# zeropoolnetwork/fawkes-crypto

Hardware: AMD Instinct MI355X
Metric: Groth16 proofs/sec + MSM scalar-muls/sec, BN254, 2^25 constraints (33552553 rows = 99.99 % of the 2^25 domain) (higher is better)
Workload: dtype u32

## Files before the change

fawkes-crypto_amd/csrc/common.hpp:

```cpp
#pragma once
#include <hip/hip_runtime.h>
#include <stdint.h>
#include <stdio.h>
#include <stdlib.h>
#include <map>
#include <string>
#include <new>
#include <stdexcept>
#include <vector>
#include <functional>
#include "../../include/fawkes_hip.h"
#include "curve.hpp"

namespace fk {

struct DevBuf {
    void *p = nullptr;
    size_t cap = 0;
    hipError_t reserve(size_t bytes) {
        if (bytes <= cap) return hipSuccess;
        if (p) { hipError_t e = hipFree(p); p = nullptr; cap = 0; if (e != hipSuccess) return e; }
        size_t want = bytes + (bytes >> 3) + 256;
        hipError_t e = hipMalloc(&p, want);
        if (e != hipSuccess) { (void)hipGetLastError(); e = hipMalloc(&p, bytes); want = bytes; }
        if (e == hipSuccess) cap = want; else { p = nullptr; (void)hipGetLastError(); }
        return e;
    }
    void release() { if (p) (void)hipFree(p); p = nullptr; cap = 0; }
    template <class T> T *as() const { return (T *)p; }
};

struct NttDomain;

struct EventPair { hipEvent_t a, b; uint64_t units; };

struct MsmLane {
    hipStream_t st = nullptr;
    hipEvent_t ev_in = nullptr;
    hipEvent_t ev_sorted = nullptr;
    bool ev_sorted_valid = false;
    DevBuf digits, sorted, totals, starts, perm, overlist, tasktab, partials, s2_cnt1, s2_seg, s2_cnt2, s2_tmp_idx, s2_tmp_lo, buckets;
    DevBuf buckets2;
    const void *last_sort_scalars = nullptr; size_t last_sort_n = 0; unsigned last_sort_c = 0; bool last_merged = false;
};

struct MsmTail {
    bool active = false;
    uint32_t cb = 0, wide = 0, W = 0, nblk = 0;
    hipEvent_t done = nullptr;
    void *h_wp = nullptr;
    size_t h_cap = 0;
    DevBuf d_wp;
};
static constexpr int MSM_TAILS = 12;
static constexpr int MSM_LANES = 4;

struct QueryIdx {
    const uint8_t *d_a_aux = nullptr, *d_b_in = nullptr, *d_b_aux = nullptr;
    const uint32_t *a = nullptr, *b = nullptr;
    uint64_t n_a = 0, n_b = 0;
};

struct KeyPre {
    void *lev = nullptr;
    size_t n = 0;
    uint32_t cb = 0, wide = 0, W = 0;
};

}

struct fk_ctx {
    int device = 0;
    hipStream_t stream = nullptr;
    std::string err;
    unsigned window_bits = 0;
    unsigned ntt_threads = 512;
    std::map<uint32_t, fk::NttDomain *> domains;
    fk::MsmLane lanes[fk::MSM_LANES];
    int lane_next = 0, lane_prev = 0;
    int co_tenants = 1;
    int lanes_in_use = fk::MSM_LANES;
    fk::MsmTail tails[fk::MSM_TAILS];
    fk::DevBuf misc;
    hipStream_t aux = nullptr;
    hipEvent_t ev_aux = nullptr, ev_main = nullptr, ev_z = nullptr;
    bool defer_back = false;
    std::vector<std::function<int()>> deferred, deferred_tails;
    bool ev_z_recorded = false;
    hipEvent_t ev_acc_done = nullptr; bool ev_acc_done_valid = false;
    bool wit_active = false;
    std::function<int()> before_block;
    bool gather_on_main = false;
    struct EarlyFront { bool done = false; int tails[4] = {-1, -1, -1, -1}; const fk_key *key = nullptr; const struct fk_r1cs_dev *r1cs = nullptr; const void *d_z = nullptr; } early;
    const fk::QueryIdx *qidx = nullptr;
    int wit_tail[4] = {-1, -1, -1, -1};
    hipStream_t copy_st = nullptr;
    struct WitSlot {
        fk::DevBuf buf; hipEvent_t ready = nullptr; bool pending = false;
        hipEvent_t part = nullptr;
        bool deferred = false; const void *host_z = nullptr; size_t host_bytes = 0;
        const fk_key *key = nullptr; const struct fk_r1cs_dev *r1cs = nullptr; uint64_t r[4], s[4];
    } wslot[2];
    int wslot_next = 0;
    hipEvent_t ev_upload_gate = nullptr;
    hipEvent_t ev_chunk[16] = {nullptr};
    fk::DevBuf ntt_s1, ntt_s2, ntt_io, hbuf, sc_a, sc_b, scan_tmp, stage_a, stage_b, stage_c, stage_z, stage_d;
    std::vector<fk::EventPair> ev_acc, ev_acc2, ev_ntt;
    std::vector<hipEvent_t> ev_pool;
    uint64_t acc_adds[2] = {0, 0};
    bool stats_on = true;
    bool debug = false;
};

struct fk_key {
    uint64_t m = 0;
    uint32_t num_input = 0, num_aux = 0;
    uint64_t n_h = 0, n_l = 0, n_a = 0, n_b = 0;
    uint32_t shard_index = 0, shard_count = 1;
    uint64_t h_lo = 0, h_hi = 0, l_lo = 0, l_hi = 0, a_lo = 0, a_hi = 0, b_lo = 0, b_hi = 0;
    uint64_t b2_lo = 0, b2_hi = 0;
// ... 173 lines not shown
```

fawkes-crypto_amd/csrc/msm.hip:

```cpp
#include "common.hpp"
#include <algorithm>
#include <string.h>
#include <type_traits>

namespace fk {

static constexpr uint32_t SEG_MAX = 4096, SEG_MIN = 256;
static constexpr uint32_t SORT_THREADS = 256;

struct MsmPlan {
    size_t n;
    uint32_t c, W, B;
    uint32_t cb, wide;
    uint32_t nchunks;
    size_t chunk;
    uint32_t cap, cap_top;
    uint32_t L, T, nblk;
    uint32_t LB, nhi, nlo;
};
#ifndef FK_S2_TILE
#define FK_S2_TILE 8192
#endif
static constexpr uint32_t S2_TILE = FK_S2_TILE;
static constexpr uint32_t S2_EPT = S2_TILE / 1024;
#ifndef FK_S1_TILE
#define FK_S1_TILE 8192
#endif
static constexpr uint32_t S1_TILE = FK_S1_TILE;
#ifndef FK_S2_MAX_HI
#define FK_S2_MAX_HI 1024
#endif
static constexpr uint32_t S2_MAX_HI = FK_S2_MAX_HI;

static MsmPlan make_plan(size_t n, unsigned forced_c, bool merged = false) {
    MsmPlan p{};
    p.n = n;
    const size_t nd = n ? n : 1;
    uint32_t lg = 0; while (((size_t)1 << (lg + 1)) <= nd + nd / 2) lg++;
    static const int t_small = tune("FK_MSM_C_SMALL", 17), t_delta = tune("FK_MSM_C_DELTA", 5), t_sig = tune("FK_MSM_CAP_SIGMA", 6), t_pre_dc = tune("FK_MSM_PRE_DC", 3);
    uint32_t c = forced_c ? forced_c : (lg >= 22 ? lg - t_delta : (lg >= 18 ? (uint32_t)t_small : (lg >= 6 ? lg - 2 : 4)));
    if (merged && !forced_c) c = (uint32_t)std::max(2, (int)c + t_pre_dc);
    if (c < 2) c = 2;
    static const uint32_t t_cmax = (uint32_t)std::min(tune("FK_MSM_C_MAX", 22), S2_MAX_HI >= 2048 ? 24 : 22);
    if (c > t_cmax) c = t_cmax;
    p.c = c;
    p.W = (255 + c - 1) / c;
    p.cb = 255 / p.W;
    p.wide = 255 - p.cb * p.W;
    if (p.wide == 0) { p.cb -= 1; p.wide = p.W; }
    c = p.cb + 1;
    p.c = c;
    p.B = 1u << (c - 1);
    size_t chunk = (n + 255) / 256;
    if (chunk < 16384) chunk = 16384;
    p.chunk = chunk;
    p.nchunks = (uint32_t)((n + chunk - 1) / chunk);
    size_t mean = nd >> (p.wide < p.W ? p.cb - 1 : p.cb);
    p.cap = (uint32_t)std::min<size_t>(2 * mean + 64, 1u << 30);
    if (t_sig > 0) { uint32_t sq = 1; while ((size_t)sq * sq < mean) sq++; p.cap = (uint32_t)std::min<size_t>(mean + (size_t)t_sig * sq + 8, 1u << 30); }
    p.cap_top = p.cap;
    static const int t_redl = tune("FK_MSM_RED_L", 0);
    p.L = p.B >= (1u << 18) ? 64 : (p.B >= (1u << 17) ? p.B / 2048 : (p.B >= 8192 ? p.B / 4096 : 1));
    if (t_redl > 0 && (uint32_t)t_redl <= p.B) p.L = (uint32_t)t_redl;
    static const int t_redl_m = tune("FK_MSM_RED_L_MERGED", 0);
    if (merged) {
        if (p.B <= (1u << 19)) p.L = std::min<uint32_t>(p.L, 8);
        else if (p.B <= (1u << 20)) p.L = std::min<uint32_t>(p.L, 16);
        if (t_redl_m > 0 && (uint32_t)t_redl_m <= p.B) p.L = (uint32_t)t_redl_m;
    }
    p.T = p.B / p.L;
    p.nblk = (p.T + 255) / 256;
    static const int t_lb = std::min(12, std::max(10, tune("FK_MSM_LB", 10)));
    p.LB = (c - 1) < (uint32_t)t_lb ? (c - 1) : (uint32_t)t_lb;
    while ((p.B >> p.LB) > S2_MAX_HI) p.LB++;
    p.nlo = 1u << p.LB;
    p.nhi = p.B >> p.LB;
    return p;
}

__global__ __launch_bounds__(256) void msm_digits_kernel(const Fr *scalars, size_t n, uint32_t cb, uint32_t wide, uint32_t W, uint32_t *digits) {
    const size_t half = (n + 1) / 2;
    const size_t i0 = (size_t)blockIdx.x * blockDim.x + threadIdx.x;
    if (i0 >= half) return;
    const size_t i1 = i0 + half;
    const bool has1 = i1 < n;
    Fr in[2];
    in[0] = scalars[i0];
    in[1] = scalars[has1 ? i1 : i0];
#pragma unroll
    for (int u = 0; u < 2; u++) {
        if (u == 1 && !has1) break;
        const size_t i = u ? i1 : i0;
        Fr s = Fr::from_mont(in[u]);
        uint32_t carry = 0;
        for (uint32_t w = 0; w < W; w++) {
            const uint32_t cw = cb + (w < wide ? 1 : 0);
            const uint32_t o = w * cb + (w < wide ? w : wide), limb = o >> 5, sh = o & 31;
            const uint32_t B = 1u << (cw - 1), mask = (1u << cw) - 1;
            uint32_t lo = limb < 8 ? s.v[limb] : 0, hi = limb + 1 < 8 ? s.v[limb + 1] : 0;
            uint32_t raw = (uint32_t)((((uint64_t)hi << 32) | lo) >> sh) & mask;
            raw += carry;
            uint32_t d, neg;
            if (raw > B) { d = (1u << cw) - raw; neg = 1; carry = 1; } else { d = raw; neg = 0; carry = 0; }
// ... 636 lines not shown
    unsigned long long extra_total = 0;
    for (int w = 0; w < 16; w++) extra_total += xsum[w];
    unsigned long long sg = ((extra_total / 2048 + 63) / 64) * 64;
    const uint32_t SEG = (uint32_t)(sg < SEG_MIN ? SEG_MIN : (sg > SEG_MAX ? SEG_MAX : sg));
    const uint32_t per = (n + 1023) / 1024, lo = tid * per, hi = lo + per < n ? lo + per : n;
    uint32_t sum = 0, heads = 0;
    for (uint32_t i = lo; i < hi && lo < n; i++) {
        const uint32_t nt = (val[i] - cap + SEG - 1) / SEG;
        val[i] = nt; sum += nt;
        heads += (i == 0 || (key[i] >> 32) != (key[i - 1] >> 32)) ? 1u : 0u;
    }
    uint32_t n_tasks, n_obs;
    uint32_t run = block_excl_scan_1024(sum, wsum, &n_tasks);
    uint32_t hrun = block_excl_scan_1024(heads, wsum, &n_obs);
    for (uint32_t i = lo; i < hi && lo < n; i++) {
        t0[i] = run; run += val[i];
        if (i == 0 || (key[i] >> 32) != (key[i - 1] >> 32)) head[hrun++] = i;
    }
    if (tid == 0) { t0[n] = n_tasks; head[n_obs] = n; }
    __syncthreads();
    if (n_tasks > max_tasks) { if (tid == 0) { dyn->error = 2; dyn->seg = SEG; dyn->n_tasks = 0; dyn->n_obs = 0; } return; }
    for (uint32_t o = tid; o < n_obs; o += 1024) {
        const uint32_t a = head[o], b = head[o + 1];
        obs[o] = OverBucket{(uint32_t)(merged ? key[a] >> 32 : key[a] & 0xffffffffu), t0[a], t0[b] - t0[a]};
    }
    for (uint32_t t = tid; t < n_tasks; t += 1024) {
        uint32_t l = 0, h = n;
        while (h - l > 1) { const uint32_t mid = (l + h) >> 1; if (t0[mid] <= t) l = mid; else h = mid; }
        tasks[t] = Task{(uint32_t)(key[l] & 0xffffffffu), t - t0[l]};
    }
    if (tid == 0) { dyn->seg = SEG; dyn->n_tasks = n_tasks; dyn->n_obs = n_obs; }
}

template <class F>
__global__ __launch_bounds__(256) void msm_bucket_reduce_kernel(const Xyzz<F> *buckets, uint32_t B, uint32_t L, uint32_t T,
                                                                uint32_t nblk, Xyzz<F> *winparts) {
    __shared__ Xyzz<F> sh[4];
    const uint32_t w = blockIdx.y;
    const uint32_t t = blockIdx.x * 256 + threadIdx.x;
    Xyzz<F> acc = Xyzz<F>::inf();
    if (t < T) {
        Xyzz<F> run = Xyzz<F>::inf();
        const Xyzz<F> *bk = buckets + (size_t)w * B + (size_t)t * L;
        for (uint32_t s = L; s-- > 0;) {
            run.add(bk[s]);
            acc.add(run);
        }
        const uint32_t k = t * L;
        if (k) {
            Xyzz<F> m = Xyzz<F>::inf();
            for (int bit = 31 - __clz(k); bit >= 0; bit--) {
                m = Xyzz<F>::dbl(m);
                if ((k >> bit) & 1) m.add(run);
            }
            acc.add(m);
        }
    }
    block_reduce_256(acc, sh);
    if (threadIdx.x == 0) winparts[(size_t)w * nblk + blockIdx.x] = acc;
}

template <class F>
__global__ __launch_bounds__(256) void msm_fold_partials_kernel(const Xyzz<F> *winparts, uint32_t nblk, Xyzz<F> *out) {
    __shared__ Xyzz<F> sh[4];
    const uint32_t w = blockIdx.x;
    Xyzz<F> acc = Xyzz<F>::inf();
    for (uint32_t b = threadIdx.x; b < nblk; b += 256) acc.add(winparts[(size_t)w * nblk + b]);
    block_reduce_256(acc, sh);
    if (threadIdx.x == 0) out[w] = acc;
}

#define FK_DBG_ST(ctx, st, name)                                                                  \
    do {                                                                                          \
        if ((ctx)->debug) {                                                                       \
            fprintf(stderr, "[fk] launch %s ...", name); fflush(stderr);                          \
            hipError_t _e = hipStreamSynchronize(st);                                             \
            fprintf(stderr, " %s\n", hipGetErrorString(_e)); fflush(stderr);                      \
        }                                                                                         \
    } while (0)

int streams_init(fk_ctx *ctx) {
    if (!ctx->copy_st) FK_HIP(ctx, hipStreamCreateWithFlags(&ctx->copy_st, hipStreamNonBlocking));
    if (!ctx->aux) {
        FK_HIP(ctx, hipStreamCreateWithFlags(&ctx->aux, hipStreamNonBlocking));
        FK_HIP(ctx, hipEventCreateWithFlags(&ctx->ev_aux, hipEventDisableTiming));
    }
    for (MsmLane &ln : ctx->lanes) {
        if (ln.st) continue;
        FK_HIP(ctx, hipStreamCreateWithFlags(&ln.st, hipStreamNonBlocking));
        FK_HIP(ctx, hipEventCreateWithFlags(&ln.ev_in, hipEventDisableTiming));
        FK_HIP(ctx, hipEventCreateWithFlags(&ln.ev_sorted, hipEventDisableTiming));
    }
    return FK_OK;
}

static int pinned_reserve(fk_ctx *ctx, void **p, size_t *cap, size_t bytes, size_t pad) {
    if (bytes + pad <= *cap) return FK_OK;
    if (*p) { FK_HIP(ctx, hipHostFree(*p)); *p = nullptr; *cap = 0; }
    FK_HIP(ctx, hipHostMalloc(p, bytes + (bytes >> 2) + pad, hipHostMallocDefault));
    *cap = bytes + (bytes >> 2) + pad;
    return FK_OK;
}

template <class F>
struct MsmJob {
    fk_ctx *ctx;
    MsmPlan p;
    MsmLane *ln;
    MsmTail *tl;
    const Affine<F> *bases, *lev;
    const Fr *scalars;
    size_t n, WB, max_tasks, max_tiles, wp_bytes;
    uint32_t WR;
    bool merged, have_sort;
    MsmDyn *dyn;
    uint32_t *digits, *sorted, *totals, *starts, *perm;
    Task *tasks;
    OverBucket *obs;
    Xyzz<F> *winparts;
};

template <class F>
static int msm_reserve(MsmJob<F> &j) {
    fk_ctx *ctx = j.ctx;
    const MsmPlan &p = j.p;
    MsmLane &ln = *j.ln;
    MsmTail &tl = *j.tl;
    const size_t n = j.n, WB = j.WB = (size_t)p.W * p.B;
    j.WR = j.merged ? 1 : p.W;
    j.wp_bytes = (size_t)j.WR * sizeof(Xyzz<F>);
    const size_t wp_dev_bytes = (size_t)j.WR * (p.nblk + 1) * sizeof(Xyzz<F>);
    const size_t max_tasks = j.max_tasks = std::max<size_t>(2048, (size_t)p.W * n / SEG_MAX) + OVER_MAX + 64;
    const uint32_t nseg = p.W * p.nhi;
    const size_t max_tiles = j.max_tiles = (size_t)p.W * ((n + S2_TILE - 1) / S2_TILE) + nseg + 1;
    struct Need { DevBuf *b; size_t bytes; };
    const Need needs[] = {
        {&ln.digits, (size_t)p.W * n * 4}, {&ln.sorted, (size_t)p.W * n * 4}, {&ln.totals, WB * 4}, {&ln.starts, WB * 4},
        {&ln.perm, WB * 4 + SIZE_BINS * 4}, {&ln.overlist, OVER_MAX * sizeof(OverEntry) + sizeof(MsmDyn) + 64}, {j.have_sort ? &ln.buckets2 : &ln.buckets, WB * sizeof(Xyzz<F>)},
        {&ln.tasktab, max_tasks * sizeof(Task) + OVER_MAX * sizeof(OverBucket) + 64}, {&ln.partials, max_tasks * sizeof(Xyzz<F>)},
        {&ln.s2_cnt1, (size_t)p.W * p.nchunks * p.nhi * 4}, {&ln.s2_seg, ((size_t)nseg * 4 + 2) * 4}, {&ln.s2_cnt2, max_tiles * p.nlo * 4},
        {&ln.s2_tmp_idx, (size_t)p.W * n * 4}, {&ln.s2_tmp_lo, (size_t)p.W * n * 2}};
    bool grow = false;
    for (const Need &nd : needs) grow = grow || nd.bytes > nd.b->cap;
    if (grow) {
        FK_HIP(ctx, hipStreamSynchronize(ln.st));
        for (const Need &nd : needs) FK_HIP(ctx, nd.b->reserve(nd.bytes));
        if (!j.have_sort) ln.last_sort_scalars = nullptr;
    }
    FK_HIP(ctx, tl.d_wp.reserve(wp_dev_bytes));
    FK_TRY(pinned_reserve(ctx, &tl.h_wp, &tl.h_cap, j.wp_bytes, 16));
    j.dyn = (MsmDyn *)((char *)ln.overlist.p + OVER_MAX * sizeof(OverEntry));
    j.tasks = ln.tasktab.as<Task>();
    j.obs = (OverBucket *)((char *)ln.tasktab.p + ((max_tasks * sizeof(Task) + 15) & ~(size_t)15));
    j.digits = ln.digits.as<uint32_t>(); j.sorted = ln.sorted.as<uint32_t>();
    j.totals = ln.totals.as<uint32_t>(); j.starts = ln.starts.as<uint32_t>();
    j.winparts = tl.d_wp.as<Xyzz<F>>();
    j.perm = ln.perm.as<uint32_t>();
    return FK_OK;
}

static void launch_scatter2(const MsmPlan &p, uint32_t n_tiles, hipStream_t st, const uint32_t *tmp_idx, const uint16_t *tmp_lo, size_t n, const uint32_t *tile_start, uint32_t nseg,
                            const uint32_t *seg_start, const uint32_t *seg_size, const uint32_t *cnt2, const uint32_t *starts, uint32_t *sorted) {
    const auto kernel = p.nlo <= 1024 ? s2_scatter2_kernel<1024> : (p.nlo <= 2048 ? s2_scatter2_kernel<2048> : s2_scatter2_kernel<4096>);
    hipLaunchKernelGGL(kernel, dim3(n_tiles), dim3(1024), 0, st, tmp_idx, tmp_lo, n, p.nhi, p.nlo, p.B, tile_start, nseg, seg_start, seg_size, cnt2, starts, sorted);
}

template <class F>
static int queue_sort(const MsmJob<F> &j) {
    fk_ctx *ctx = j.ctx;
    const MsmPlan &p = j.p;
    MsmLane &ln = *j.ln;
    hipStream_t st = ln.st;
// ... 35 lines not shown
    uint32_t *totals = j.totals, *perm = j.perm, *size_bins = perm + WB;
    unsigned long long *d_adds = &dyn->adds;
    static const int t_many = tune("FK_MSM_OVER_MANY", 2048);
    const uint32_t many = (uint32_t)std::min<size_t>(std::max<size_t>((size_t)t_many, WB / 8192), OVER_MAX - 64);
    hipLaunchKernelGGL(msm_cap_kernel, dim3(1), dim3(64), 0, st, dyn, p.cap ? p.cap : 1u, many);
    hipLaunchKernelGGL(msm_over_list_kernel, dim3((unsigned)((WB + 255) / 256)), dim3(256), 0, st, totals, WB, ln.overlist.as<OverEntry>(), dyn);
    hipLaunchKernelGGL(msm_tasks_kernel, dim3(1), dim3(1024), 0, st, ln.overlist.as<OverEntry>(), dyn, p.B, j.merged ? 1 : 0, j.tasks, (uint32_t)j.max_tasks, j.obs);
    FK_HIP(ctx, hipMemsetAsync(size_bins, 0, SIZE_BINS * 4, st));
    if (j.merged) {
        uint32_t *mt = perm + p.B;
        hipLaunchKernelGGL(msm_merge_totals_kernel, dim3(std::min<uint32_t>((p.B + 255) / 256, 1024)), dim3(256), 0, st, totals, p.B, p.W, dyn, mt, d_adds);
        hipLaunchKernelGGL(msm_size_hist_kernel, dim3((unsigned)std::min<size_t>((p.B + 255) / 256, 1024)), dim3(256), 0, st, mt, (size_t)p.B, dyn, p.W, size_bins, (unsigned long long *)nullptr);
        hipLaunchKernelGGL(msm_size_scan_kernel, dim3(1), dim3(SIZE_BINS), 0, st, size_bins);
        hipLaunchKernelGGL(msm_size_scatter_kernel, dim3((unsigned)((p.B + 1023) / 1024)), dim3(1024), 0, st, mt, (size_t)p.B, dyn, p.W, size_bins, perm);
    } else {
        hipLaunchKernelGGL(msm_size_hist_kernel, dim3((unsigned)std::min<size_t>((WB + 255) / 256, 1024)), dim3(256), 0, st, totals, WB, dyn, 1u, size_bins, d_adds);
        hipLaunchKernelGGL(msm_size_scan_kernel, dim3(1), dim3(SIZE_BINS), 0, st, size_bins);
        hipLaunchKernelGGL(msm_size_scatter_kernel, dim3((unsigned)((WB + 1023) / 1024)), dim3(1024), 0, st, totals, WB, dyn, 1u, size_bins, perm);
    }
    FK_HIP(ctx, hipGetLastError());
    FK_DBG_ST(ctx, st, "msm_size_order");
    if (ctx->debug) {
        MsmDyn h{};
        FK_HIP(ctx, hipMemcpy(&h, dyn, sizeof h, hipMemcpyDeviceToHost));
        fprintf(stderr, "[fk] msm n=%zu c=%u (W=%u: %u x %u bits + %u x %u bits) cap=%u (plan %u): %u oversized buckets, %u tasks of %u entries, %u fold groups\n", j.n, p.c,
                p.W, p.wide, p.cb + 1, p.W - p.wide, p.cb, h.cap, p.cap, h.n_over, h.n_tasks, h.seg, h.n_obs);
        fflush(stderr);
    }
    return FK_OK;
}

template <class F>
static Xyzz<F> *bucket_buf(const MsmJob<F> &j) { return (j.have_sort ? j.ln->buckets2 : j.ln->buckets).template as<Xyzz<F>>(); }

template <class F>
static int queue_accumulate(MsmJob<F> j) {
    fk_ctx *ctx = j.ctx;
    const MsmPlan &p = j.p;
    hipStream_t st = j.ln->st;
    constexpr int MINW = std::is_same<F, Fq>::value ? 4 : 2;
    Xyzz<F> *buckets = bucket_buf(j);
    std::vector<EventPair> &evv = (sizeof(F) == sizeof(Fq)) ? ctx->ev_acc : ctx->ev_acc2;
    FK_TRY(stats_begin(ctx, evv, (uint64_t)j.n, st));
    if (j.merged)
        hipLaunchKernelGGL(HIP_KERNEL_NAME(msm_accumulate_merged_kernel<F, MINW>), dim3((p.B + 255) / 256), dim3(256), 0, st, j.bases, j.lev, j.sorted, j.n,
                           j.starts, j.totals, p.B, p.W, j.dyn, j.perm, j.perm + p.B, buckets);
    else
        hipLaunchKernelGGL(HIP_KERNEL_NAME(msm_accumulate_kernel<F, MINW>), dim3((unsigned)((j.WB + 255) / 256)), dim3(256), 0, st, j.bases, j.sorted, j.n,
                           j.starts, j.totals, p.B, p.W, j.dyn, j.perm, buckets);
    FK_HIP(ctx, hipGetLastError());
    FK_TRY(stats_end(ctx, evv, st));
    if (!ctx->ev_acc_done) FK_HIP(ctx, hipEventCreateWithFlags(&ctx->ev_acc_done, hipEventDisableTiming));
    FK_HIP(ctx, hipEventRecord(ctx->ev_acc_done, st)); ctx->ev_acc_done_valid = true;
    FK_DBG_ST(ctx, st, "msm_accumulate");
    return FK_OK;
}

template <class F>
static int queue_tail(MsmJob<F> j) {
    using FC = typename ColdOf<F>::type;
    fk_ctx *ctx = j.ctx;
    const MsmPlan &p = j.p;
    MsmLane &ln = *j.ln;
    MsmTail &tl = *j.tl;
    hipStream_t st = ln.st;
    Xyzz<F> *buckets = bucket_buf(j);
    hipLaunchKernelGGL(HIP_KERNEL_NAME(msm_overflow_kernel<F, FC>), dim3(2048), dim3(64), 0, st,
                       j.bases, j.lev, j.sorted, j.n, j.starts, j.totals, p.B, j.dyn, j.tasks, ln.partials.as<Xyzz<FC>>());
    FK_HIP(ctx, hipGetLastError());
    FK_DBG_ST(ctx, st, "msm_overflow");
    hipLaunchKernelGGL(HIP_KERNEL_NAME(msm_overflow_fold_kernel<F>), dim3(256), dim3(256), 0, st, j.obs, j.dyn, ln.partials.as<Xyzz<F>>(), buckets);
    FK_HIP(ctx, hipGetLastError());
    FK_DBG_ST(ctx, st, "msm_overflow_fold");
    hipLaunchKernelGGL(HIP_KERNEL_NAME(msm_bucket_reduce_kernel<F>), dim3(p.nblk, j.WR), dim3(256), 0, st, buckets, p.B, p.L, p.T, p.nblk, j.winparts);
    Xyzz<F> *folded = j.winparts + (size_t)j.WR * p.nblk;
    hipLaunchKernelGGL(HIP_KERNEL_NAME(msm_fold_partials_kernel<F>), dim3(j.WR), dim3(256), 0, st, j.winparts, p.nblk, folded);
    FK_HIP(ctx, hipGetLastError());
    FK_HIP(ctx, hipMemcpyAsync(tl.h_wp, folded, j.wp_bytes, hipMemcpyDeviceToHost, st));
    FK_HIP(ctx, hipMemcpyAsync((char *)tl.h_wp + j.wp_bytes, &j.dyn->adds, 8, hipMemcpyDeviceToHost, st));
    FK_HIP(ctx, hipMemcpyAsync((char *)tl.h_wp + j.wp_bytes + 8, &j.dyn->error, 4, hipMemcpyDeviceToHost, st));
    FK_HIP(ctx, hipEventRecord(tl.done, st));
    FK_DBG_ST(ctx, st, "msm_bucket_reduce");
    return FK_OK;
}

template <class F>
static int msm_begin(fk_ctx *ctx, const Affine<F> *d_bases, const Fr *d_scalars, size_t n, bool reuse_sort, int *tail_out, hipEvent_t ready, const KeyPre *pre = nullptr) {
    *tail_out = -1;
    if (n == 0) return FK_OK;
    if (n >= ((size_t)1 << 31)) FK_SET_ERR(ctx, FK_ERR_BAD_ARG, "msm: n too large");
    int ti = -1;
    for (int i = 0; i < MSM_TAILS; i++) if (!ctx->tails[i].active) { ti = i; break; }
    if (ti < 0) FK_SET_ERR(ctx, FK_ERR_BAD_ARG, "msm: too many outstanding multiplications");
    MsmTail &tl = ctx->tails[ti];
    if (!tl.done) FK_HIP(ctx, hipEventCreateWithFlags(&tl.done, hipEventDisableTiming));
    MsmPlan p = make_plan(n, ctx->window_bits);
    bool merged = false;
    if (pre && pre->lev && pre->n == n) {
        const MsmPlan pm = make_plan(n, ctx->window_bits, true);
        if (pm.cb == pre->cb && pm.wide == pre->wide && pm.W == pre->W) { p = pm; merged = true; }
    }
    MsmLane &prev = ctx->lanes[ctx->lane_prev];
    const bool have_sort = reuse_sort && prev.st && prev.last_sort_scalars == (const void *)d_scalars && prev.last_sort_n == n && prev.last_sort_c == p.c && prev.last_merged == merged;
    const int li = have_sort ? ctx->lane_prev : ctx->lane_next;
    MsmLane &ln = ctx->lanes[li];
    if (!ln.st) FK_SET_ERR(ctx, FK_ERR_HIP, "msm: the context's streams were not created");
    static const int t_lanes = tune("FK_MSM_LANES", 0);
    const int n_lanes = (t_lanes >= 1 && t_lanes <= MSM_LANES && !ctx->defer_back && ctx->deferred.empty())
                            ? t_lanes : (ctx->lanes_in_use >= 2 && ctx->lanes_in_use <= MSM_LANES ? ctx->lanes_in_use : MSM_LANES);
    ctx->lane_prev = li; ctx->lane_next = (li + 1) % n_lanes;
    if (ready) FK_HIP(ctx, hipStreamWaitEvent(ln.st, ready, 0));
    else {
        FK_HIP(ctx, hipEventRecord(ln.ev_in, ctx->stream));
        FK_HIP(ctx, hipStreamWaitEvent(ln.st, ln.ev_in, 0));
    }
    MsmJob<F> job{};
    job.ctx = ctx; job.p = p; job.ln = &ln; job.tl = &tl;
    job.bases = d_bases; job.lev = merged ? (const Affine<F> *)pre->lev : nullptr; job.scalars = d_scalars;
    job.n = n; job.merged = merged; job.have_sort = have_sort;
    FK_TRY(msm_reserve(job));
    if (!have_sort) {
        FK_TRY(queue_sort(job));
        FK_TRY(queue_size_order(job));
        FK_HIP(ctx, hipEventRecord(ln.ev_sorted, ln.st)); ln.ev_sorted_valid = true;
    }
    tl.active = true; tl.cb = p.cb; tl.wide = p.wide; tl.W = job.WR; tl.nblk = 1;
    *tail_out = ti;
    if (ctx->defer_back) {
        ctx->deferred.push_back([job] { return queue_accumulate<F>(job); });
        ctx->deferred_tails.push_back([job] { return queue_tail<F>(job); });
        return FK_OK;
    }
    FK_TRY(queue_accumulate<F>(job));
    return queue_tail<F>(job);
}

int msm_run_deferred(fk_ctx *ctx, hipEvent_t after) {
    if (after) for (MsmLane &ln : ctx->lanes) if (ln.st) FK_HIP(ctx, hipStreamWaitEvent(ln.st, after, 0));
    std::vector<std::function<int()>> accs, tails;
    accs.swap(ctx->deferred); tails.swap(ctx->deferred_tails);
    for (auto &f : accs) FK_TRY(f());
    for (auto &f : tails) FK_TRY(f());
    return FK_OK;
}

template <class F>
static int msm_end(fk_ctx *ctx, int tail, Xyzz<F> *out) {
    *out = Xyzz<F>::inf();
    if (tail < 0) return FK_OK;
    if (tail >= MSM_TAILS || !ctx->tails[tail].active) FK_SET_ERR(ctx, FK_ERR_BAD_ARG, "msm: bad tail handle");
    MsmTail &tl = ctx->tails[tail];
    tl.active = false;
    FK_HIP(ctx, hipEventSynchronize(tl.done));
    const Xyzz<F> *wp = (const Xyzz<F> *)tl.h_wp;
    { const char *extra = (const char *)tl.h_wp + (size_t)tl.W * tl.nblk * sizeof(Xyzz<F>);
      uint64_t adds; uint32_t err;
      memcpy(&adds, extra, 8); memcpy(&err, extra + 8, 4);
      ctx->acc_adds[sizeof(F) == sizeof(Fq) ? 0 : 1] += adds;
      if (err) FK_SET_ERR(ctx, FK_ERR_HIP, "msm: the oversized-bucket tables overflowed (%s)", err == 1 ? "more than OVER_MAX buckets above the cap" : "more segment tasks than the bound"); }
    Xyzz<F> acc = Xyzz<F>::inf();
    for (uint32_t w = tl.W; w-- > 0;) {
        const uint32_t cw = tl.cb + (w < tl.wide ? 1 : 0);
        for (uint32_t k = 0; k < cw; k++) acc = Xyzz<F>::dbl(acc);
        for (uint32_t b = 0; b < tl.nblk; b++) acc.add(wp[(size_t)w * tl.nblk + b]);
    }
    *out = acc;
    if (ctx->debug) { fprintf(stderr, "[fk] msm host horner done\n"); fflush(stderr); }
    return FK_OK;
}

int msm_sync(fk_ctx *ctx) {
    if (ctx->aux) FK_HIP(ctx, hipStreamSynchronize(ctx->aux));
    for (MsmLane &ln : ctx->lanes) if (ln.st) FK_HIP(ctx, hipStreamSynchronize(ln.st));
    return FK_OK;
}

void msm_abandon(fk_ctx *ctx) {
    ctx->wit_active = false;
    ctx->early.done = false;
    ctx->defer_back = false; ctx->deferred.clear(); ctx->deferred_tails.clear();
    if (ctx->aux) (void)hipStreamSynchronize(ctx->aux);
    for (int i = 0; i < MSM_TAILS; i++) ctx->tails[i].active = false;
    for (MsmLane &ln : ctx->lanes) { if (ln.st) (void)hipStreamSynchronize(ln.st); ln.last_sort_scalars = nullptr; }
}

void msm_release(fk_ctx *ctx) {
    if (ctx->aux) { (void)hipStreamSynchronize(ctx->aux); (void)hipStreamDestroy(ctx->aux); ctx->aux = nullptr; }
    if (ctx->ev_aux) { (void)hipEventDestroy(ctx->ev_aux); ctx->ev_aux = nullptr; }
    if (ctx->ev_main) { (void)hipEventDestroy(ctx->ev_main); ctx->ev_main = nullptr; }
    if (ctx->ev_z) { (void)hipEventDestroy(ctx->ev_z); ctx->ev_z = nullptr; }
    if (ctx->ev_upload_gate) { (void)hipEventDestroy(ctx->ev_upload_gate); ctx->ev_upload_gate = nullptr; }
    for (hipEvent_t &e : ctx->ev_chunk) if (e) { (void)hipEventDestroy(e); e = nullptr; }
    if (ctx->ev_acc_done) { (void)hipEventDestroy(ctx->ev_acc_done); ctx->ev_acc_done = nullptr; ctx->ev_acc_done_valid = false; }
    for (MsmLane &ln : ctx->lanes) {
        if (ln.st) (void)hipStreamSynchronize(ln.st);
        for (DevBuf *b : {&ln.digits, &ln.sorted, &ln.totals, &ln.starts, &ln.perm, &ln.overlist, &ln.tasktab, &ln.partials, &ln.s2_cnt1, &ln.s2_seg,
                          &ln.s2_cnt2, &ln.s2_tmp_idx, &ln.s2_tmp_lo, &ln.buckets, &ln.buckets2})
            b->release();
        if (ln.ev_in) (void)hipEventDestroy(ln.ev_in);
        if (ln.ev_sorted) (void)hipEventDestroy(ln.ev_sorted);
        if (ln.st) (void)hipStreamDestroy(ln.st);
        ln = MsmLane();
    }
    for (int i = 0; i < MSM_TAILS; i++) {
        MsmTail &tl = ctx->tails[i];
        if (tl.done) (void)hipEventDestroy(tl.done);
        if (tl.h_wp) (void)hipHostFree(tl.h_wp);
        tl.d_wp.release();
        tl = MsmTail();
    }
}

int msm_g1_begin(fk_ctx *ctx, const G1Affine *d_bases, const Fr *d_scalars, size_t n, int *tail, hipEvent_t ready, const KeyPre *pre) {
    return msm_begin<Fq>(ctx, d_bases, d_scalars, n, false, tail, ready, pre);
}
int msm_g1_end(fk_ctx *ctx, int tail, G1Xyzz *out) { return msm_end<Fq>(ctx, tail, out); }
int msm_g2_begin(fk_ctx *ctx, const G2Affine *d_bases, const Fr *d_scalars, size_t n, bool reuse_sort, int *tail, hipEvent_t ready, const KeyPre *pre) {
    return msm_begin<Fq2>(ctx, d_bases, d_scalars, n, reuse_sort, tail, ready, pre);
}
int msm_g2_end(fk_ctx *ctx, int tail, G2Xyzz *out) { return msm_end<Fq2>(ctx, tail, out); }

template <class F>
static int msm_run(fk_ctx *ctx, const Affine<F> *d_bases, const Fr *d_scalars, size_t n, Xyzz<F> *out, bool reuse_sort = false, const KeyPre *pre = nullptr) {
    int tail = -1;
    *out = Xyzz<F>::inf();
    FK_TRY(msm_begin<F>(ctx, d_bases, d_scalars, n, reuse_sort, &tail, nullptr, pre));
    return msm_end<F>(ctx, tail, out);
}

// ... 24 lines not shown
                 (double)bytes / (double)(1ull << 30), (double)fr / (double)(1ull << 30));
        if (require) { ctx->err = std::string(msg) + " and FK_MSM_PRECOMP=require"; return FK_ERR_OOM; }
        ctx->err += (ctx->err.empty() ? "warning: " : "; ") + std::string(msg) + " -- that array takes the slower W-bucket-set path";
        return FK_OK;
    }
    const Affine<F> *prev = d_bases;
    for (uint32_t w = 1; w < p.W; w++) {
        Affine<F> *cur = (Affine<F> *)lev + (size_t)(w - 1) * n;
        const uint32_t bits = p.cb + ((w - 1) < p.wide ? 1 : 0);
        constexpr int NB = sizeof(F) == sizeof(Fq) ? 4 : 2;
        hipLaunchKernelGGL(HIP_KERNEL_NAME(msm_level_kernel<F, NB>), dim3((unsigned)(((n + NB - 1) / NB + 255) / 256)), dim3(256), 0, ctx->stream, prev, n, bits, cur);
        prev = cur;
    }
    if (hipGetLastError() != hipSuccess || hipStreamSynchronize(ctx->stream) != hipSuccess) { (void)hipFree(lev); FK_SET_ERR(ctx, FK_ERR_HIP, "msm: level precomputation failed"); }
    out->lev = lev; out->n = n; out->cb = p.cb; out->wide = p.wide; out->W = p.W;
    return FK_OK;
}

void key_pre_free(fk_key *k) {
    for (KeyPre *p : {&k->pre_h, &k->pre_l, &k->pre_a, &k->pre_b1, &k->pre_b2}) { if (p->lev) (void)hipFree(p->lev); *p = KeyPre(); }
}

static size_t proof_scratch_still_needed(fk_ctx *ctx, const fk_key *k) {
    const size_t pts = (size_t)(k->h_hi - k->h_lo) + (k->l_hi - k->l_lo) + (k->a_hi - k->a_lo) + std::max(k->b_hi - k->b_lo, k->b2_hi - k->b2_lo);
    const size_t nv = (size_t)k->num_input + k->num_aux;
    const size_t nmax = std::max<size_t>(std::max<size_t>(k->h_hi - k->h_lo, k->l_hi - k->l_lo), std::max<size_t>(k->a_hi - k->a_lo, std::max(k->b_hi - k->b_lo, k->b2_hi - k->b2_lo)));
    const MsmPlan pl = make_plan(nmax, ctx->window_bits, true);
    const size_t lane_fixed = (size_t)pl.W * pl.B * (MSM_LANES * (sizeof(Xyzz<Fq>) + 16) + sizeof(Xyzz<Fq2>)) + ((size_t)1 << 30);
    const uint64_t h_held = k->h_hi - k->h_lo;
    const size_t quot = h_held == 0 ? 0 : h_held >= k->n_h ? (size_t)k->m * 32 * (6 + 10) : (size_t)k->m * 32 * 6 + (size_t)k->m / k->shard_count * 32 * 10;
    const size_t need = pts * 14 * 13 + lane_fixed + quot + 2 * nv * 32;
    size_t have = 0;
    for (const MsmLane &ln : ctx->lanes)
        for (const DevBuf *b : {&ln.digits, &ln.sorted, &ln.totals, &ln.starts, &ln.perm, &ln.overlist, &ln.tasktab, &ln.partials, &ln.s2_cnt1, &ln.s2_seg,
                                &ln.s2_cnt2, &ln.s2_tmp_idx, &ln.s2_tmp_lo, &ln.buckets, &ln.buckets2}) have += b->cap;
    for (const DevBuf *b : {&ctx->ntt_s1, &ctx->ntt_s2, &ctx->ntt_io, &ctx->hbuf, &ctx->sc_a, &ctx->sc_b, &ctx->stage_a, &ctx->stage_b, &ctx->stage_c, &ctx->stage_z,
                            &ctx->stage_d, &ctx->wslot[0].buf, &ctx->wslot[1].buf}) have += b->cap;
    return (need > have ? need - have : 0) * (size_t)std::max(1, ctx->co_tenants);
}

int key_levels_headroom(fk_ctx *ctx, const fk_key *k, int64_t *bytes) {
    size_t fr = 0, tot = 0;
    FK_HIP(ctx, hipMemGetInfo(&fr, &tot));
    *bytes = (int64_t)fr - (int64_t)proof_scratch_still_needed(ctx, k) - ((int64_t)2 << 30);
    return FK_OK;
}

int key_precompute(fk_ctx *ctx, fk_key *k) {
    const char *e = getenv("FK_MSM_PRECOMP");
    const bool require = e && !strcmp(e, "require");
    const int on = e && !require ? atoi(e) : 1;
    key_pre_free(k);
    ctx->err.clear();
    if (!on) return FK_OK;
    const size_t reserve = proof_scratch_still_needed(ctx, k) + ((size_t)8 << 30);
    struct Cand { const char *name; int which; size_t n, bytes; double worth; };
    std::vector<Cand> cand;
    const bool b_shared = k->b2_lo == k->b_lo && k->b2_hi == k->b_hi && k->d_b1 && k->d_b2;
    auto level_bytes = [&](size_t n, size_t pt) -> size_t {
        const char *e2 = getenv("FK_MSM_PRE_MIN_LOG2");
        const int min_lg = e2 ? atoi(e2) : 21;
        if (min_lg < 6 || min_lg > 40 || n + n / 2 < ((size_t)1 << min_lg)) return 0;
        const MsmPlan p = make_plan(n, ctx->window_bits, true);
        return p.W < 2 ? 0 : (size_t)(p.W - 1) * n * pt;
    };
    auto add_cand = [&](const char *name, int which, const void *d, size_t n, size_t pt, double w) {
        const size_t b = d ? level_bytes(n, pt) : 0;
// ... 215 lines not shown
```

fawkes-crypto_amd/csrc/prover.hip:

```cpp
#include <execinfo.h>
#include <signal.h>
#include <unistd.h>
#include "common.hpp"
#include <chrono>
#include <mutex>
#include <string.h>
#include <stdlib.h>

using namespace fk;

namespace fk {

int stats_begin(fk_ctx *ctx, std::vector<EventPair> &v, uint64_t units, hipStream_t st) {
    if (!ctx->stats_on) return FK_OK;
    if (v.size() >= 4096) {
        for (auto &old : v) { ctx->ev_pool.push_back(old.a); ctx->ev_pool.push_back(old.b); }
        v.clear();
    }
    EventPair ep{};
    ep.units = units;
    for (hipEvent_t *e : {&ep.a, &ep.b}) {
        if (!ctx->ev_pool.empty()) { *e = ctx->ev_pool.back(); ctx->ev_pool.pop_back(); }
        else FK_HIP(ctx, hipEventCreate(e));
    }
// ... 6 lines not shown
    FK_HIP(ctx, hipEventRecord(v.back().b, st ? st : ctx->stream));
    return FK_OK;
}

static void g1_to_raw(uint8_t out[64], const G1Xyzz &p) { G1Affine a = p.to_affine(); memcpy(out, &a, 64); }
static void g2_to_raw(uint8_t out[128], const G2Xyzz &p) { G2Affine a = p.to_affine(); memcpy(out, &a, 128); }
static G1Affine g1_from_raw(const uint8_t *b) { G1Affine a; memcpy(&a, b, 64); return a; }
static G2Affine g2_from_raw(const uint8_t *b) { G2Affine a; memcpy(&a, b, 128); return a; }

static void slice(uint64_t n, uint32_t idx, uint32_t cnt, uint64_t *lo, uint64_t *hi) {
    *lo = (uint64_t)((unsigned __int128)n * idx / cnt);
    *hi = (uint64_t)((unsigned __int128)n * (idx + 1) / cnt);
}

static double now_ms() {
    return std::chrono::duration<double, std::milli>(std::chrono::steady_clock::now().time_since_epoch()).count();
}

}

static_assert(sizeof(G1Affine) == 64 && sizeof(G2Affine) == 128 && sizeof(Fr) == 32, "raw layouts");

extern "C" {

int fk_init(int device_id, fk_ctx **out) {
    if (!out) return FK_ERR_BAD_ARG;
    *out = nullptr;
    int ndev = 0;
    if (hipGetDeviceCount(&ndev) != hipSuccess || ndev <= 0) return FK_ERR_HIP;
    if (device_id < 0 || device_id >= ndev) return FK_ERR_BAD_ARG;
    if (hipSetDevice(device_id) != hipSuccess) return FK_ERR_HIP;
    fk_ctx *ctx = new fk_ctx();
    ctx->device = device_id;
    { const char *d = getenv("FK_DEBUG"); ctx->debug = d && d[0] && d[0] != '0'; }
    { const char *t = getenv("FK_CO_TENANTS"); if (t) { const int v = atoi(t); if (v >= 1 && v <= 64) ctx->co_tenants = v; } }
    if (ctx->debug || getenv("FK_BACKTRACE")) {
        static std::once_flag once;
        std::call_once(once, [] {
            void *warm[4];
            (void)backtrace(warm, 4);
            static struct sigaction prev_segv, prev_abrt;
            auto h = +[](int sig, siginfo_t *info, void *uctx) {
                void *bt[64];
                const int n = backtrace(bt, 64);
                const char msg[] = "[fk] fatal signal, native backtrace:\n";
                (void)!write(2, msg, sizeof msg - 1);
                backtrace_symbols_fd(bt, n, 2);
                const struct sigaction &prev = sig == SIGSEGV ? prev_segv : prev_abrt;
                if ((prev.sa_flags & SA_SIGINFO) && prev.sa_sigaction) { prev.sa_sigaction(sig, info, uctx); return; }
                if (!(prev.sa_flags & SA_SIGINFO) && prev.sa_handler != SIG_DFL && prev.sa_handler != SIG_IGN && prev.sa_handler) { prev.sa_handler(sig); return; }
                signal(sig, SIG_DFL); raise(sig);
            };
            struct sigaction sa;
            memset(&sa, 0, sizeof sa);
            sa.sa_sigaction = h;
            sa.sa_flags = SA_SIGINFO | SA_ONSTACK;
            sigemptyset(&sa.sa_mask);
            sigaction(SIGSEGV, &sa, &prev_segv);
            sigaction(SIGABRT, &sa, &prev_abrt);
        });
    }
    { const int v = tune("FK_NTT_THREADS", 512); if (v == 64 || v == 128 || v == 256 || v == 512 || v == 1024) ctx->ntt_threads = (unsigned)v; }
    if (hipStreamCreate(&ctx->stream) != hipSuccess) { delete ctx; return FK_ERR_HIP; }
    if (streams_init(ctx) != FK_OK) { fk_free(ctx); return FK_ERR_HIP; }
    *out = ctx;
    return FK_OK;
// ... 980 lines not shown
```

Baseline: 4.414.

## Restructure MSM bucket reduction with block scans and CU-aware segment length

Bucket reduction now performs a block-level suffix scan of running sums. Each thread multiplies its running sum by the constant L instead of by t*L, which removes the per-thread scalar multiplication by a large index. The fold kernel is rewritten to combine per-block partial pairs hierarchically. The segment length L is now derived from the device CU count and total bucket work rather than fixed thresholds. The overflow kernel moves out of the deferred tail so it runs right after sorting, using a separate partials buffer per sort state, and deferred accumulate and tail are merged into one closure. This may change the overlap between lanes and adds extra buffer memory.

```diff
diff --git a/fawkes-crypto_amd/csrc/common.hpp b/fawkes-crypto_amd/csrc/common.hpp
--- a/fawkes-crypto_amd/csrc/common.hpp
+++ b/fawkes-crypto_amd/csrc/common.hpp
@@ -40,7 +40,7 @@
     hipEvent_t ev_sorted = nullptr;
     bool ev_sorted_valid = false;
     DevBuf digits, sorted, totals, starts, perm, overlist, tasktab, partials, s2_cnt1, s2_seg, s2_cnt2, s2_tmp_idx, s2_tmp_lo, buckets;
-    DevBuf buckets2;
+    DevBuf buckets2, partials2;
     const void *last_sort_scalars = nullptr; size_t last_sort_n = 0; unsigned last_sort_c = 0; bool last_merged = false;
 };
 
@@ -71,6 +71,7 @@
 
 struct fk_ctx {
     int device = 0;
+    int num_cu = 256;
     hipStream_t stream = nullptr;
     std::string err;
     unsigned window_bits = 0;
@@ -85,7 +86,7 @@
     hipStream_t aux = nullptr;
     hipEvent_t ev_aux = nullptr, ev_main = nullptr, ev_z = nullptr;
     bool defer_back = false;
-    std::vector<std::function<int()>> deferred, deferred_tails;
+    std::vector<std::function<int()>> deferred;
     bool ev_z_recorded = false;
     hipEvent_t ev_acc_done = nullptr; bool ev_acc_done_valid = false;
     bool wit_active = false;
diff --git a/fawkes-crypto_amd/csrc/msm.hip b/fawkes-crypto_amd/csrc/msm.hip
--- a/fawkes-crypto_amd/csrc/msm.hip
+++ b/fawkes-crypto_amd/csrc/msm.hip
@@ -32,7 +32,7 @@
 #endif
 static constexpr uint32_t S2_MAX_HI = FK_S2_MAX_HI;
 
-static MsmPlan make_plan(size_t n, unsigned forced_c, bool merged = false) {
+static MsmPlan make_plan(size_t n, unsigned forced_c, bool merged = false, int num_cu = 0) {
     MsmPlan p{};
     p.n = n;
     const size_t nd = n ? n : 1;
@@ -60,15 +60,13 @@
     if (t_sig > 0) { uint32_t sq = 1; while ((size_t)sq * sq < mean) sq++; p.cap = (uint32_t)std::min<size_t>(mean + (size_t)t_sig * sq + 8, 1u << 30); }
     p.cap_top = p.cap;
     static const int t_redl = tune("FK_MSM_RED_L", 0);
-    p.L = p.B >= (1u << 18) ? 64 : (p.B >= (1u << 17) ? p.B / 2048 : (p.B >= 8192 ? p.B / 4096 : 1));
+    {
+        const uint64_t lanes = (uint64_t)(num_cu ? num_cu : 256) * 256, all = (uint64_t)p.B * (merged ? 1 : p.W);
+        p.L = 1;
+        while (p.L < 64 && p.L < p.B && all > lanes * p.L) p.L <<= 1;
+    }
     if (t_redl > 0 && (uint32_t)t_redl <= p.B) p.L = (uint32_t)t_redl;
-    static const int t_redl_m = tune("FK_MSM_RED_L_MERGED", 0);
-    if (merged) {
-        if (p.B <= (1u << 19)) p.L = std::min<uint32_t>(p.L, 8);
-        else if (p.B <= (1u << 20)) p.L = std::min<uint32_t>(p.L, 16);
-        if (t_redl_m > 0 && (uint32_t)t_redl_m <= p.B) p.L = (uint32_t)t_redl_m;
-    }
-    p.T = p.B / p.L;
+    p.T = (p.B + p.L - 1) / p.L;
     p.nblk = (p.T + 255) / 256;
     static const int t_lb = std::min(12, std::max(10, tune("FK_MSM_LB", 10)));
     p.LB = (c - 1) < (uint32_t)t_lb ? (c - 1) : (uint32_t)t_lb;
@@ -771,40 +769,75 @@
     if (tid == 0) { dyn->seg = SEG; dyn->n_tasks = n_tasks; dyn->n_obs = n_obs; }
 }
 
+
+template <class F>
+static __device__ __forceinline__ Xyzz<F> mul_small(const Xyzz<F> &p, uint32_t k) {
+    Xyzz<F> m = Xyzz<F>::inf();
+    if (!k) return m;
+#pragma unroll 1
+    for (int bit = 31 - __clz(k); bit >= 0; bit--) {
+        m = Xyzz<F>::dbl(m);
+        if ((k >> bit) & 1) m.add(p);
+    }
+    return m;
+}
+
+template <class F>
+static __device__ __forceinline__ void block_suffix_scan_256(Xyzz<F> &v, Xyzz<F> *sh) {
+    const uint32_t lane = threadIdx.x & 63, wv = threadIdx.x >> 6;
+#pragma unroll 1
+    for (int off = 1; off < 64; off <<= 1) {
+        Xyzz<F> o = shfl_down_obj(v, off);
+        if (lane + (uint32_t)off < 64) v.add(o);
+    }
+    if (lane == 0) sh[wv] = v;
+    __syncthreads();
+#pragma unroll 1
+    for (uint32_t k = 3; k > wv; k--) { Xyzz<F> o = sh[k]; v.add(o); }
+    __syncthreads();
+}
+
 template <class F>
 __global__ __launch_bounds__(256) void msm_bucket_reduce_kernel(const Xyzz<F> *buckets, uint32_t B, uint32_t L, uint32_t T,
                                                                 uint32_t nblk, Xyzz<F> *winparts) {
     __shared__ Xyzz<F> sh[4];
     const uint32_t w = blockIdx.y;
     const uint32_t t = blockIdx.x * 256 + threadIdx.x;
-    Xyzz<F> acc = Xyzz<F>::inf();
+    Xyzz<F> acc = Xyzz<F>::inf(), run = Xyzz<F>::inf();
     if (t < T) {
-        Xyzz<F> run = Xyzz<F>::inf();
-        const Xyzz<F> *bk = buckets + (size_t)w * B + (size_t)t * L;
-        for (uint32_t s = L; s-- > 0;) {
+        const size_t s0 = (size_t)t * L;
+        const uint32_t cnt = s0 + L <= B ? L : (uint32_t)(B - s0);
+        const Xyzz<F> *bk = buckets + (size_t)w * B + s0;
+#pragma unroll 1
+        for (uint32_t s = cnt; s-- > 0;) {
             run.add(bk[s]);
             acc.add(run);
         }
-        const uint32_t k = t * L;
-        if (k) {
-            Xyzz<F> m = Xyzz<F>::inf();
-            for (int bit = 31 - __clz(k); bit >= 0; bit--) {
-                m = Xyzz<F>::dbl(m);
-                if ((k >> bit) & 1) m.add(run);
-            }
-            acc.add(m);
-        }
-    }
+    }
+    block_suffix_scan_256(run, sh);
+    Xyzz<F> *out = winparts + ((size_t)w * nblk + blockIdx.x) * 2;
+    if (threadIdx.x == 0) out[1] = run;
+    else { const Xyzz<F> m = mul_small(run, L); acc.add(m); }
     block_reduce_256(acc, sh);
-    if (threadIdx.x == 0) winparts[(size_t)w * nblk + blockIdx.x] = acc;
-}
-
-template <class F>
-__global__ __launch_bounds__(256) void msm_fold_partials_kernel(const Xyzz<F> *winparts, uint32_t nblk, Xyzz<F> *out) {
+    if (threadIdx.x == 0) out[0] = acc;
+}
+
+template <class F>
+__global__ __launch_bounds__(256) void msm_fold_partials_kernel(const Xyzz<F> *winparts, uint32_t nblk, uint32_t L, Xyzz<F> *out) {
     __shared__ Xyzz<F> sh[4];
-    const uint32_t w = blockIdx.x;
-    Xyzz<F> acc = Xyzz<F>::inf();
-    for (uint32_t b = threadIdx.x; b < nblk; b += 256) acc.add(winparts[(size_t)w * nblk + b]);
+    const uint32_t w = blockIdx.x, per = (nblk + 255) / 256, b0 = threadIdx.x * per;
+    const Xyzz<F> *wp = winparts + (size_t)w * nblk * 2;
+    Xyzz<F> acc = Xyzz<F>::inf(), run = Xyzz<F>::inf(), q = Xyzz<F>::inf();
+    const uint32_t cnt = b0 >= nblk ? 0 : (b0 + per <= nblk ? per : nblk - b0);
+#pragma unroll 1
+    for (uint32_t j = cnt; j-- > 0;) {
+        acc.add(wp[(size_t)(b0 + j) * 2]);
+        if (j + 1 < cnt) q.add(run);
+        run.add(wp[(size_t)(b0 + j) * 2 + 1]);
+    }
+    block_suffix_scan_256(run, sh);
+    if (threadIdx.x) { const Xyzz<F> m = mul_small(run, per); q.add(m); }
+    { const Xyzz<F> m = mul_small(q, 256u * L); acc.add(m); }
     block_reduce_256(acc, sh);
     if (threadIdx.x == 0) out[w] = acc;
 }
@@ -868,7 +901,7 @@
     const size_t n = j.n, WB = j.WB = (size_t)p.W * p.B;
     j.WR = j.merged ? 1 : p.W;
     j.wp_bytes = (size_t)j.WR * sizeof(Xyzz<F>);
-    const size_t wp_dev_bytes = (size_t)j.WR * (p.nblk + 1) * sizeof(Xyzz<F>);
+    const size_t wp_dev_bytes = (size_t)j.WR * (2 * p.nblk + 1) * sizeof(Xyzz<F>);
     const size_t max_tasks = j.max_tasks = std::max<size_t>(2048, (size_t)p.W * n / SEG_MAX) + OVER_MAX + 64;
     const uint32_t nseg = p.W * p.nhi;
     const size_t max_tiles = j.max_tiles = (size_t)p.W * ((n + S2_TILE - 1) / S2_TILE) + nseg + 1;
@@ -876,7 +909,7 @@
     const Need needs[] = {
         {&ln.digits, (size_t)p.W * n * 4}, {&ln.sorted, (size_t)p.W * n * 4}, {&ln.totals, WB * 4}, {&ln.starts, WB * 4},
         {&ln.perm, WB * 4 + SIZE_BINS * 4}, {&ln.overlist, OVER_MAX * sizeof(OverEntry) + sizeof(MsmDyn) + 64}, {j.have_sort ? &ln.buckets2 : &ln.buckets, WB * sizeof(Xyzz<F>)},
-        {&ln.tasktab, max_tasks * sizeof(Task) + OVER_MAX * sizeof(OverBucket) + 64}, {&ln.partials, max_tasks * sizeof(Xyzz<F>)},
+        {&ln.tasktab, max_tasks * sizeof(Task) + OVER_MAX * sizeof(OverBucket) + 64}, {j.have_sort ? &ln.partials2 : &ln.partials, max_tasks * sizeof(Xyzz<F>)},
         {&ln.s2_cnt1, (size_t)p.W * p.nchunks * p.nhi * 4}, {&ln.s2_seg, ((size_t)nseg * 4 + 2) * 4}, {&ln.s2_cnt2, max_tiles * p.nlo * 4},
         {&ln.s2_tmp_idx, (size_t)p.W * n * 4}, {&ln.s2_tmp_lo, (size_t)p.W * n * 2}};
     bool grow = false;
@@ -978,6 +1011,20 @@
 
 template <class F>
 static Xyzz<F> *bucket_buf(const MsmJob<F> &j) { return (j.have_sort ? j.ln->buckets2 : j.ln->buckets).template as<Xyzz<F>>(); }
+template <class F>
+static Xyzz<F> *partials_buf(const MsmJob<F> &j) { return (j.have_sort ? j.ln->partials2 : j.ln->partials).template as<Xyzz<F>>(); }
+
+template <class F>
+static int queue_overflow(const MsmJob<F> &j) {
+    using FC = typename ColdOf<F>::type;
+    fk_ctx *ctx = j.ctx;
+    hipStream_t st = j.ln->st;
+    hipLaunchKernelGGL(HIP_KERNEL_NAME(msm_overflow_kernel<F, FC>), dim3(2048), dim3(64), 0, st,
+                       j.bases, j.lev, j.sorted, j.n, j.starts, j.totals, j.p.B, j.dyn, j.tasks, reinterpret_cast<Xyzz<FC> *>(partials_buf(j)));
+    FK_HIP(ctx, hipGetLastError());
+    FK_DBG_ST(ctx, st, "msm_overflow");
+    return FK_OK;
+}
 
 template <class F>
 static int queue_accumulate(MsmJob<F> j) {
@@ -1004,23 +1051,17 @@
 
 template <class F>
 static int queue_tail(MsmJob<F> j) {
-    using FC = typename ColdOf<F>::type;
     fk_ctx *ctx = j.ctx;
     const MsmPlan &p = j.p;
-    MsmLane &ln = *j.ln;
     MsmTail &tl = *j.tl;
-    hipStream_t st = ln.st;
+    hipStream_t st = j.ln->st;
     Xyzz<F> *buckets = bucket_buf(j);
-    hipLaunchKernelGGL(HIP_KERNEL_NAME(msm_overflow_kernel<F, FC>), dim3(2048), dim3(64), 0, st,
-                       j.bases, j.lev, j.sorted, j.n, j.starts, j.totals, p.B, j.dyn, j.tasks, ln.partials.as<Xyzz<FC>>());
-    FK_HIP(ctx, hipGetLastError());
-    FK_DBG_ST(ctx, st, "msm_overflow");
-    hipLaunchKernelGGL(HIP_KERNEL_NAME(msm_overflow_fold_kernel<F>), dim3(256), dim3(256), 0, st, j.obs, j.dyn, ln.partials.as<Xyzz<F>>(), buckets);
+    hipLaunchKernelGGL(HIP_KERNEL_NAME(msm_overflow_fold_kernel<F>), dim3(256), dim3(256), 0, st, j.obs, j.dyn, partials_buf(j), buckets);
     FK_HIP(ctx, hipGetLastError());
     FK_DBG_ST(ctx, st, "msm_overflow_fold");
     hipLaunchKernelGGL(HIP_KERNEL_NAME(msm_bucket_reduce_kernel<F>), dim3(p.nblk, j.WR), dim3(256), 0, st, buckets, p.B, p.L, p.T, p.nblk, j.winparts);
-    Xyzz<F> *folded = j.winparts + (size_t)j.WR * p.nblk;
-    hipLaunchKernelGGL(HIP_KERNEL_NAME(msm_fold_partials_kernel<F>), dim3(j.WR), dim3(256), 0, st, j.winparts, p.nblk, folded);
+    Xyzz<F> *folded = j.winparts + (size_t)j.WR * p.nblk * 2;
+    hipLaunchKernelGGL(HIP_KERNEL_NAME(msm_fold_partials_kernel<F>), dim3(j.WR), dim3(256), 0, st, j.winparts, p.nblk, p.L, folded);
     FK_HIP(ctx, hipGetLastError());
     FK_HIP(ctx, hipMemcpyAsync(tl.h_wp, folded, j.wp_bytes, hipMemcpyDeviceToHost, st));
     FK_HIP(ctx, hipMemcpyAsync((char *)tl.h_wp + j.wp_bytes, &j.dyn->adds, 8, hipMemcpyDeviceToHost, st));
@@ -1040,10 +1081,10 @@
     if (ti < 0) FK_SET_ERR(ctx, FK_ERR_BAD_ARG, "msm: too many outstanding multiplications");
     MsmTail &tl = ctx->tails[ti];
     if (!tl.done) FK_HIP(ctx, hipEventCreateWithFlags(&tl.done, hipEventDisableTiming));
-    MsmPlan p = make_plan(n, ctx->window_bits);
+    MsmPlan p = make_plan(n, ctx->window_bits, false, ctx->num_cu);
     bool merged = false;
     if (pre && pre->lev && pre->n == n) {
-        const MsmPlan pm = make_plan(n, ctx->window_bits, true);
+        const MsmPlan pm = make_plan(n, ctx->window_bits, true, ctx->num_cu);
         if (pm.cb == pre->cb && pm.wide == pre->wide && pm.W == pre->W) { p = pm; merged = true; }
     }
     MsmLane &prev = ctx->lanes[ctx->lane_prev];
@@ -1070,11 +1111,11 @@
         FK_TRY(queue_size_order(job));
         FK_HIP(ctx, hipEventRecord(ln.ev_sorted, ln.st)); ln.ev_sorted_valid = true;
     }
+    FK_TRY(queue_overflow(job));
     tl.active = true; tl.cb = p.cb; tl.wide = p.wide; tl.W = job.WR; tl.nblk = 1;
     *tail_out = ti;
     if (ctx->defer_back) {
-        ctx->deferred.push_back([job] { return queue_accumulate<F>(job); });
-        ctx->deferred_tails.push_back([job] { return queue_tail<F>(job); });
+        ctx->deferred.push_back([job] { FK_TRY(queue_accumulate<F>(job)); return queue_tail<F>(job); });
         return FK_OK;
     }
     FK_TRY(queue_accumulate<F>(job));
@@ -1083,10 +1124,9 @@
 
 int msm_run_deferred(fk_ctx *ctx, hipEvent_t after) {
     if (after) for (MsmLane &ln : ctx->lanes) if (ln.st) FK_HIP(ctx, hipStreamWaitEvent(ln.st, after, 0));
-    std::vector<std::function<int()>> accs, tails;
-    accs.swap(ctx->deferred); tails.swap(ctx->deferred_tails);
-    for (auto &f : accs) FK_TRY(f());
-    for (auto &f : tails) FK_TRY(f());
+    std::vector<std::function<int()>> backs;
+    backs.swap(ctx->deferred);
+    for (auto &f : backs) FK_TRY(f());
     return FK_OK;
 }
 
@@ -1124,7 +1164,7 @@
 void msm_abandon(fk_ctx *ctx) {
     ctx->wit_active = false;
     ctx->early.done = false;
-    ctx->defer_back = false; ctx->deferred.clear(); ctx->deferred_tails.clear();
+    ctx->defer_back = false; ctx->deferred.clear();
     if (ctx->aux) (void)hipStreamSynchronize(ctx->aux);
     for (int i = 0; i < MSM_TAILS; i++) ctx->tails[i].active = false;
     for (MsmLane &ln : ctx->lanes) { if (ln.st) (void)hipStreamSynchronize(ln.st); ln.last_sort_scalars = nullptr; }
@@ -1140,7 +1180,7 @@
     if (ctx->ev_acc_done) { (void)hipEventDestroy(ctx->ev_acc_done); ctx->ev_acc_done = nullptr; ctx->ev_acc_done_valid = false; }
     for (MsmLane &ln : ctx->lanes) {
         if (ln.st) (void)hipStreamSynchronize(ln.st);
-        for (DevBuf *b : {&ln.digits, &ln.sorted, &ln.totals, &ln.starts, &ln.perm, &ln.overlist, &ln.tasktab, &ln.partials, &ln.s2_cnt1, &ln.s2_seg,
+        for (DevBuf *b : {&ln.digits, &ln.sorted, &ln.totals, &ln.starts, &ln.perm, &ln.overlist, &ln.tasktab, &ln.partials, &ln.partials2, &ln.s2_cnt1, &ln.s2_seg,
                           &ln.s2_cnt2, &ln.s2_tmp_idx, &ln.s2_tmp_lo, &ln.buckets, &ln.buckets2})
             b->release();
         if (ln.ev_in) (void)hipEventDestroy(ln.ev_in);
@@ -1231,7 +1271,7 @@
     const size_t need = pts * 14 * 13 + lane_fixed + quot + 2 * nv * 32;
     size_t have = 0;
     for (const MsmLane &ln : ctx->lanes)
-        for (const DevBuf *b : {&ln.digits, &ln.sorted, &ln.totals, &ln.starts, &ln.perm, &ln.overlist, &ln.tasktab, &ln.partials, &ln.s2_cnt1, &ln.s2_seg,
+        for (const DevBuf *b : {&ln.digits, &ln.sorted, &ln.totals, &ln.starts, &ln.perm, &ln.overlist, &ln.tasktab, &ln.partials, &ln.partials2, &ln.s2_cnt1, &ln.s2_seg,
                                 &ln.s2_cnt2, &ln.s2_tmp_idx, &ln.s2_tmp_lo, &ln.buckets, &ln.buckets2}) have += b->cap;
     for (const DevBuf *b : {&ctx->ntt_s1, &ctx->ntt_s2, &ctx->ntt_io, &ctx->hbuf, &ctx->sc_a, &ctx->sc_b, &ctx->stage_a, &ctx->stage_b, &ctx->stage_c, &ctx->stage_z,
                             &ctx->stage_d, &ctx->wslot[0].buf, &ctx->wslot[1].buf}) have += b->cap;
diff --git a/fawkes-crypto_amd/csrc/prover.hip b/fawkes-crypto_amd/csrc/prover.hip
--- a/fawkes-crypto_amd/csrc/prover.hip
+++ b/fawkes-crypto_amd/csrc/prover.hip
@@ -62,6 +62,7 @@
     if (hipSetDevice(device_id) != hipSuccess) return FK_ERR_HIP;
     fk_ctx *ctx = new fk_ctx();
     ctx->device = device_id;
+    { int cu = 0; if (hipDeviceGetAttribute(&cu, hipDeviceAttributeMultiprocessorCount, device_id) == hipSuccess && cu > 0) ctx->num_cu = cu; }
     { const char *d = getenv("FK_DEBUG"); ctx->debug = d && d[0] && d[0] != '0'; }
     { const char *t = getenv("FK_CO_TENANTS"); if (t) { const int v = atoi(t); if (v >= 1 && v <= 64) ctx->co_tenants = v; } }
     if (ctx->debug || getenv("FK_BACKTRACE")) {
```

Result: no change. 4.396 (-0.4%).
